# jhultman/vision3d

Hardware: AMD Instinct MI355X
Metric: frames/sec SECOND fwd, 16k-pt KITTI cloud (higher is better)
Workload: dtype f16x3-scaled (fp32-class): fp32 operands split into f16 hi + lo pieces of x * s under per-tensor power-of-two scales, 3 MFMA terms (lo*hi + hi*lo + hi*hi), fp32 accumulate; relative product error 2^-22 -- the result differs from the reference's fp32 modules by fp32 summation noise: strict elementwis

## Files before the change

### vision3d_amd/csrc/dense_conv.hip

```cpp
#include "v3d_internal.h"
#include "split_prec.h"

typedef unsigned short bf16_t;

#define DC_BM 64
#define DC_BN 128
#define DC_KC 32
#define DC_THREADS 256

template <int PREC>
__global__ void dc_pack_weights_kernel(const float* __restrict__ w, const float* __restrict__ scale, int Cout, int Cin,
                                       int ks, int CoutPad, bf16_t* __restrict__ img) {
  const int taps = ks * ks, chunks = Cin / DC_KC;
  const long long total = (long long)taps * chunks * (CoutPad / 16) * 4 * 16 * 8;
  float sw = 1.f;
  if constexpr (PREC == 1) sw = v3d_wimg_weight_scale(reinterpret_cast<unsigned*>(img + total * 2));
  for (long long t = (long long)blockIdx.x * blockDim.x + threadIdx.x; t < total; t += (long long)gridDim.x * blockDim.x) {
    long long r = t;
    const int e = (int)(r % 8); r /= 8;
    const int j = (int)(r % 16); r /= 16;
    const int kg = (int)(r % 4); r /= 4;
    const int nf = (int)(r % (CoutPad / 16)); r /= (CoutPad / 16);
    const int chunk = (int)(r % chunks); r /= chunks;
    const int tap = (int)r;
// ... 481 lines not shown
#endif
#if DL_TIMELINE
__device__ unsigned long long dl_tl[2][64];
extern "C" int v3d_debug_dense_timeline(unsigned long long* host_out) {
  return (int)hipMemcpyFromSymbol(host_out, HIP_SYMBOL(dl_tl), sizeof(dl_tl));
}
#define DL_STAMP(role, idx) do { if (blockIdx.x == 8 && lane == 0 && (wave == 0 || wave == 4)) dl_tl[role][idx] = __builtin_readcyclecounter(); } while (0)
#else
#define DL_STAMP(role, idx)
#endif

__device__ __attribute__((aligned(16))) const unsigned dl_zero16[4] = {0u, 0u, 0u, 0u};

template <int KS, int MT, int PREC>
__device__ __forceinline__ void dl_tile(unsigned char* smem_l, const bf16_t* __restrict__ x_hi, const bf16_t* __restrict__ x_lo,
                                        const bf16_t* __restrict__ w_img, const float* __restrict__ bias, const DcParams& p,
                                        bf16_t* __restrict__ y_hi, bf16_t* __restrict__ y_lo, float* __restrict__ y_nchw,
                                        const int mtile) {
  constexpr int BM = MT * 16, A_PLANE = BM * DL_KC * 2, STAGE = 2 * A_PLANE;
  const int tid = threadIdx.x, lane = tid & 63;
  const int wave = __builtin_amdgcn_readfirstlane(tid >> 6);
  const bool loader = wave >= 4;
  const int m0 = mtile * BM;
  const int n0 = blockIdx.y * DC_BN;
  if (p.occ) {
    const int R = p.reach, wpr = (p.W + 31) >> 5, span = 2 * R + 1;
    const int mlast = min(m0 + BM, p.M) - 1;
    const int r0 = m0 / p.W, r1 = mlast / p.W;
    const int per_seg = span * wpr, total = (r1 - r0 + 1) * per_seg;
    bool near_any = false;
    for (int q = lane; q < total; q += 64) {
      const int seg = q / per_seg, rem = q - seg * per_seg, dy = rem / wpr - R, wd = rem % wpr;
      const int r = r0 + seg, rr = r + dy;
      if (rr < 0 || rr >= p.B * p.H || rr / p.H != r / p.H) continue;
      const int xs = (r == r0 ? m0 - r0 * p.W : 0) - R, xe = (r == r1 ? mlast - r1 * p.W : p.W - 1) + R;
      const int lo = max(xs, wd * 32), hi = min(min(xe, p.W - 1), wd * 32 + 31);
      if (lo > hi) continue;
      const unsigned mask = (0xFFFFFFFFu >> (31 - (hi - wd * 32))) & (0xFFFFFFFFu << (lo - wd * 32));
      near_any |= (~p.occ[(size_t)rr * wpr + wd] & mask) != 0u;
    }
    if (!__builtin_amdgcn_readfirstlane(__ballot(near_any) != 0ull)) {
      if (p.tile_state) {
        if (p.tile_state[mtile] == 0u) return;
        __syncthreads();
        if (tid == 0) p.tile_state[mtile] = 0u;
      }
      const int HW = p.H * p.W, parts = (min(p.cout_store, n0 + DC_BN) - n0) >> 3;
      for (int q = tid; q < BM * parts; q += DL_THREADS) {
        const int row = q / parts, part = q - row * parts;
        const int m = m0 + row;
        if (m >= p.M) break;
        const size_t src = (size_t)(m % HW) * p.cout_store + n0 + part * 8, dst = (size_t)m * p.cout_store + n0 + part * 8;
        *reinterpret_cast<u32x4*>(y_hi + dst) = *reinterpret_cast<const u32x4*>(p.bg_hi + src);
        *reinterpret_cast<u32x4*>(y_lo + dst) = *reinterpret_cast<const u32x4*>(p.bg_lo + src);
      }
      return;
    }
  }
  if (p.tile_state && tid == 0) p.tile_state[mtile] = 1u;
  const int chunks = (p.Cin + DL_KC - 1) / DL_KC;
  const int stages = KS * KS * chunks;
  auto a_slot = [](int px, int part) { return px * 256 + ((part ^ (px & 15)) << 4); };

  f32x4 acc[MT][2];
#pragma unroll
  for (int i = 0; i < MT; i++) {
    acc[i][0] = f32x4{0.f, 0.f, 0.f, 0.f};
    acc[i][1] = f32x4{0.f, 0.f, 0.f, 0.f};
  }

  if (loader) {
    const int lw = wave - 4;
    const int sub = lane >> 4, slot = lane & 15;
    int a_pix[MT], a_hw[MT];
    {
      const int m = m0 + lw * MT * 4 + sub;
      const int b = m / (p.H * p.W), rem = m - b * p.H * p.W;
      int h = rem / p.W, w = rem - h * p.W;
#pragma unroll
      for (int j = 0; j < MT; j++) {
        const int mj = m + 4 * j;
        a_pix[j] = mj < p.M ? mj : -1;
        a_hw[j] = mj < p.M ? ((h << 16) | w) : 0;
        w += 4;
        if (w >= p.W) {
          w -= p.W;
          if (++h == p.H) h = 0;
        }
      }
    }
    typedef const __attribute__((address_space(1))) void* gptr_t;
    typedef __attribute__((address_space(3))) void* lptr_t;
    int tap = 0, chunk = 0;
    auto gather = [&](int buf) {
      const int dy = KS == 3 ? tap / 3 - 1 : 0, dx = KS == 3 ? tap % 3 - 1 : 0;
      unsigned char* A = smem_l + buf * STAGE + lw * MT * 1024;
#pragma unroll
      for (int j = 0; j < MT; j++) {
        const int px = (lw * MT + j) * 4 + sub;
        const int ch = chunk * DL_KC + ((slot ^ (px & 15)) << 3);
        const int hh = (a_hw[j] >> 16) + dy, ww = (a_hw[j] & 0xFFFF) + dx;
        const bool ok = a_pix[j] >= 0 && hh >= 0 && hh < p.H && ww >= 0 && ww < p.W && ch < p.Cin;
        const size_t off = (size_t)(a_pix[j] + dy * p.W + dx) * p.Cin + ch;
        const bf16_t* sh = ok ? x_hi + off : reinterpret_cast<const bf16_t*>(dl_zero16);
        const bf16_t* sl = ok ? x_lo + off : reinterpret_cast<const bf16_t*>(dl_zero16);
        __builtin_amdgcn_global_load_lds((gptr_t)sh, (lptr_t)(A + j * 1024), 16, 0, 0);
        __builtin_amdgcn_global_load_lds((gptr_t)sl, (lptr_t)(A + A_PLANE + j * 1024), 16, 0, 0);
      }
      if (++chunk == chunks) {
        chunk = 0;
        ++tap;
      }
    };
    DL_STAMP(1, 0);
    gather(0);
    DL_STAMP(1, 1);
    __syncthreads();
    DL_STAMP(1, 2);
    for (int s = 0; s < stages; s++) {
      if (s + 1 < stages) gather((s + 1) & 1);
      if (s < 8) DL_STAMP(1, 3 + 2 * s);
      __syncthreads();
      if (s < 8) DL_STAMP(1, 4 + 2 * s);
    }
    DL_STAMP(1, 30);
  } else {
    const size_t plane_elems = (size_t)(p.CoutPad / 16) * 4 * 16 * 8;
    u32x4 cb[DL_SS][4];
    int tap = 0, chunk = 0;
    auto load_b = [&](int ss) {
      const int steps32 = p.Cin / DC_KC;
      const size_t step = (size_t)tap * steps32 + min(chunk * DL_SS + ss, steps32 - 1);
      const bf16_t* wb = w_img + step * 2 * plane_elems + ((size_t)(n0 / 16 + wave * 2) * 64 + lane) * 8;
#pragma unroll
      for (int nt2 = 0; nt2 < 2; nt2++) {
        cb[ss][nt2 * 2 + 0] = *reinterpret_cast<const u32x4*>(wb + (size_t)nt2 * 512);
        cb[ss][nt2 * 2 + 1] = *reinterpret_cast<const u32x4*>(wb + plane_elems + (size_t)nt2 * 512);
      }
    };
    auto next_stage = [&]() {
      if (++chunk == chunks) {
        chunk = 0;
        ++tap;
      }
    };
    auto multiply = [&](int buf, bool more, bool stamp) {
      const unsigned char* A = smem_l + buf * STAGE;
      constexpr int NSTEP = DL_SS * MT / 2;
      u32x4 fh[3][2], fl[3][2];
      auto frag = [&](int t, u32x4& h, u32x4& l) {
        const int ss = t / MT, i = t % MT;
        const int off = a_slot(i * 16 + (lane & 15), ss * 4 + (lane >> 4));
        h = *reinterpret_cast<const u32x4*>(A + off);
        l = *reinterpret_cast<const u32x4*>(A + A_PLANE + off);
      };
      frag(0, fh[0][0], fl[0][0]);
      frag(1, fh[0][1], fl[0][1]);
      frag(2, fh[1][0], fl[1][0]);
      frag(3, fh[1][1], fl[1][1]);
#pragma unroll
      for (int u = 0; u < NSTEP; u++) {
        if (u + 2 < NSTEP) {
          frag(2 * u + 4, fh[(u + 2) % 3][0], fl[(u + 2) % 3][0]);
          frag(2 * u + 5, fh[(u + 2) % 3][1], fl[(u + 2) % 3][1]);
        }
        const int t0 = 2 * u, t1 = 2 * u + 1;
        const int s0 = t0 / MT, i0 = t0 % MT, s1 = t1 / MT, i1 = t1 % MT;
        const u32x4 b0h0 = cb[s0][0], b0l0 = cb[s0][1];
        const u32x4 b0h1 = cb[s0][2], b0l1 = cb[s0][3];
        const u32x4 b1h0 = cb[s1][0], b1l0 = cb[s1][1];
        const u32x4 b1h1 = cb[s1][2], b1l1 = cb[s1][3];
        const u32x4 a0h = fh[u % 3][0], a0l = fl[u % 3][0], a1h = fh[u % 3][1], a1l = fl[u % 3][1];
        acc[i0][0] = split_mfma<PREC>(a0l, b0h0, acc[i0][0]);
        acc[i0][1] = split_mfma<PREC>(a0l, b0h1, acc[i0][1]);
        acc[i1][0] = split_mfma<PREC>(a1l, b1h0, acc[i1][0]);
        acc[i1][1] = split_mfma<PREC>(a1l, b1h1, acc[i1][1]);
        __builtin_amdgcn_sched_barrier(0);
        acc[i0][0] = split_mfma<PREC>(a0h, b0l0, acc[i0][0]);
        acc[i0][1] = split_mfma<PREC>(a0h, b0l1, acc[i0][1]);
        acc[i1][0] = split_mfma<PREC>(a1h, b1l0, acc[i1][0]);
        acc[i1][1] = split_mfma<PREC>(a1h, b1l1, acc[i1][1]);
        __builtin_amdgcn_sched_barrier(0);
        acc[i0][0] = split_mfma<PREC>(a0h, b0h0, acc[i0][0]);
        acc[i0][1] = split_mfma<PREC>(a0h, b0h1, acc[i0][1]);
        acc[i1][0] = split_mfma<PREC>(a1h, b1h0, acc[i1][0]);
        acc[i1][1] = split_mfma<PREC>(a1h, b1h1, acc[i1][1]);
        if (i0 == MT - 1) load_b(s0);
        if (i1 == MT - 1) load_b(s1);
        __builtin_amdgcn_sched_barrier(0);
#if DL_TIMELINE
        if (stamp && (u == 0 || u == 1 || u == 8 || u == 16 || u == 17)) DL_STAMP(0, 40 + u);
#endif
      }
    };
    DL_STAMP(0, 0);
#pragma unroll
    for (int ss = 0; ss < DL_SS; ss++) load_b(ss);
    if (stages > 1) next_stage();
    DL_STAMP(0, 1);
    __syncthreads();
    DL_STAMP(0, 2);
    for (int s = 0; s < stages; s++) {
      const bool more = s + 1 < stages;
      multiply(s & 1, more, s == 3);
      if (s + 2 < stages) next_stage();
      if (s < 8) DL_STAMP(0, 3 + 2 * s);
      __syncthreads();
      if (s < 8) DL_STAMP(0, 4 + 2 * s);
    }
    DL_STAMP(0, 30);
  }

  DL_STAMP(loader ? 1 : 0, 31);
  const DcScales sc = dc_scales<PREC>(p);
  float vmax = 0.f;
  float* tile = reinterpret_cast<float*>(smem_l);
  f32x4 eb0 = f32x4{0.f, 0.f, 0.f, 0.f}, eb1 = eb0;
  {
    const int co = n0 + (tid & 15) * 8;
    if (bias && y_hi && co < p.cout_store) {
      eb0 = *reinterpret_cast<const f32x4*>(bias + co);
      eb1 = *reinterpret_cast<const f32x4*>(bias + co + 4);
    }
  }
  if (!loader) {
#pragma unroll
    for (int i = 0; i < MT; i++)
#pragma unroll
      for (int j = 0; j < 2; j++)
#pragma unroll
        for (int r = 0; r < 4; r++) {
          const int row = i * 16 + (lane >> 4) * 4 + r;
          const int col = wave * 32 + j * 16 + (lane & 15);
          tile[row * DL_TS + col] = acc[i][j][r];
        }
  }
  __syncthreads();
  DL_STAMP(loader ? 1 : 0, 32);
  if (y_hi) {
    const int c8 = tid & 15, co = n0 + c8 * 8;
    if (co < p.cout_store) {
#pragma unroll
      for (int k = 0; k < (BM + 31) / 32; k++) {
        const int row = (tid >> 4) + 32 * k;
        const int m = m0 + row;
        if (row < BM && m < p.M) {
          const f32x4 t0 = *reinterpret_cast<const f32x4*>(tile + row * DL_TS + c8 * 8);
          const f32x4 t1 = *reinterpret_cast<const f32x4*>(tile + row * DL_TS + c8 * 8 + 4);
          float v[8] = {dc_finish<PREC>(t0[0], eb0[0], sc), dc_finish<PREC>(t0[1], eb0[1], sc), dc_finish<PREC>(t0[2], eb0[2], sc),
                        dc_finish<PREC>(t0[3], eb0[3], sc), dc_finish<PREC>(t1[0], eb1[0], sc), dc_finish<PREC>(t1[1], eb1[1], sc),
                        dc_finish<PREC>(t1[2], eb1[2], sc), dc_finish<PREC>(t1[3], eb1[3], sc)};
          u32x4 vh, vl;
#pragma unroll
          for (int e2 = 0; e2 < 4; e2++) {
            float v0 = v[2 * e2], v1 = v[2 * e2 + 1];
            if (p.relu) {
              v0 = fmaxf(v0, 0.f);
              v1 = fmaxf(v1, 0.f);
            }
            if constexpr (PREC == 1) vmax = fmaxf(vmax, fmaxf(fabsf(v0), fabsf(v1)));
            unsigned h, l;
            split_pair<PREC>(v0, v1, sc.s_out, h, l);
            vh[e2] = h;
            vl[e2] = l;
          }
          *reinterpret_cast<u32x4*>(y_hi + (size_t)m * p.cout_store + co) = vh;
          *reinterpret_cast<u32x4*>(y_lo + (size_t)m * p.cout_store + co) = vl;
        }
      }
    }
    if constexpr (PREC == 1) dc_range_check(p, vmax, sc.limit);
  }
  if (y_nchw) {
    const int HW = p.H * p.W;
    for (int q = tid; q < (BM / 4) * DC_BN; q += DL_THREADS) {
      const int col = q / (BM / 4), r4 = q % (BM / 4);
      const int co = n0 + col;
      if (co >= p.cout_store) continue;
      const float bv = bias ? bias[co] : 0.f;
#pragma unroll
      for (int e = 0; e < 4; e++) {
        const int m = m0 + r4 * 4 + e;
        if (m >= p.M) continue;
        float v = dc_finish<PREC>(tile[(r4 * 4 + e) * DL_TS + col], bv, sc);
        if (p.relu) v = fmaxf(v, 0.f);
        const int b = m / HW, pix = m - b * HW;
        y_nchw[((size_t)b * p.cout_store + co) * HW + pix] = v;
      }
    }
  }
  DL_STAMP(loader ? 1 : 0, 33);
}

#define D2_TH 5
#define D2_TW 16
#define D2_HW (D2_TW + 2)
#define D2_HALO ((D2_TH + 2) * D2_HW)
#define D2_PIECES ((D2_HALO + 7) / 8)
#define D2_HALF (D2_PIECES * 1024)
#define D2_PLANE (2 * D2_HALF)
static_assert(2 * D2_PLANE <= dl_smem(D2_TH), "the neighbourhood image lives in the tile kernel's LDS request");
static_assert(D2_TH * 16 * DL_TS * 4 <= 2 * D2_PLANE, "the epilogue tile reuses the image's LDS");
#define D2_THREADS 256
template <int PREC>
__device__ __forceinline__ bool dl_tile2d(unsigned char* smem_l, const bf16_t* __restrict__ x_hi, const bf16_t* __restrict__ x_lo,
                                          const bf16_t* __restrict__ w_img, const float* __restrict__ bias, const DcParams& p,
                                          bf16_t* __restrict__ y_hi, bf16_t* __restrict__ y_lo, const int mtile, int* s_next) {
  constexpr int MT = D2_TH, BM = MT * 16, NT = D2_THREADS;
  const int tid = threadIdx.x, lane = tid & 63;
  const int wave = __builtin_amdgcn_readfirstlane(tid >> 6);
  const int tx_n = (p.W + D2_TW - 1) / D2_TW, ty_n = (p.H + D2_TH - 1) / D2_TH;
  const int b = mtile / (ty_n * tx_n), rt = mtile - b * ty_n * tx_n;
  const int y0 = (rt / tx_n) * D2_TH, x0 = (rt % tx_n) * D2_TW;
  if (p.occ) {
    const int R = p.reach, wpr = (p.W + 31) >> 5;
    const int ylo = max(y0 - R, 0), yhi = min(min(y0 + D2_TH - 1, p.H - 1) + R, p.H - 1);
    const int xlo = max(x0 - R, 0), xhi = min(min(x0 + D2_TW - 1, p.W - 1) + R, p.W - 1);
    const int w0 = xlo >> 5, nw = (xhi >> 5) - w0 + 1, total = (yhi - ylo + 1) * nw;
    const unsigned in_place = p.tile_state ? p.tile_state[mtile] : 1u;
    bool near_any = false;
    for (int q = lane; q < total; q += 64) {
      const int row = ylo + q / nw, wd = w0 + q % nw;
      const int lo = max(xlo, wd * 32), hi = min(xhi, wd * 32 + 31);
      const unsigned mask = (0xFFFFFFFFu >> (31 - (hi - wd * 32))) & (0xFFFFFFFFu << (lo - wd * 32));
      near_any |= (~p.occ[((size_t)b * p.H + row) * wpr + wd] & mask) != 0u;
    }
    if (!__builtin_amdgcn_readfirstlane(__ballot(near_any) != 0ull)) {
      if (p.tile_state) {
        if (in_place == 0u) return false;
        __syncthreads();
        if (tid == 0) p.tile_state[mtile] = 0u;
      }
      const int parts = p.cout_store >> 3;
      for (int q = tid; q < BM * parts; q += NT) {
        const int row = q / parts, part = q - row * parts;
        const int yy = y0 + (row >> 4), xx = x0 + (row & 15);
        if (yy >= p.H || xx >= p.W) continue;
        const size_t src = ((size_t)yy * p.W + xx) * p.cout_store + part * 8, dst = (((size_t)b * p.H + yy) * p.W + xx) * p.cout_store + part * 8;
        *reinterpret_cast<u32x4*>(y_hi + dst) = *reinterpret_cast<const u32x4*>(p.bg_hi + src);
        *reinterpret_cast<u32x4*>(y_lo + dst) = *reinterpret_cast<const u32x4*>(p.bg_lo + src);
      }
      return false;
    }
  }
  if (p.tile_state && tid == 0) p.tile_state[mtile] = 1u;

  f32x4 acc[MT][2];
#pragma unroll
  for (int i = 0; i < MT; i++) {
    acc[i][0] = f32x4{0.f, 0.f, 0.f, 0.f};
    acc[i][1] = f32x4{0.f, 0.f, 0.f, 0.f};
  }
  {
    const int plane = wave & 1, half = wave >> 1;
    const int sub = lane >> 3, slot = lane & 7;
    const bf16_t* xp = plane ? x_lo : x_hi;
    typedef const __attribute__((address_space(1))) void* gptr_t;
    typedef __attribute__((address_space(3))) void* lptr_t;
    unsigned char* dstb = smem_l + plane * D2_PLANE + half * D2_HALF;
#pragma unroll
    for (int j = 0; j < D2_PIECES; j++) {
      const int hp = j * 8 + sub;
      const int hy = hp / D2_HW, hx = hp - hy * D2_HW;
      const int yy = y0 - 1 + hy, xx = x0 - 1 + hx;
      const bool ok = hp < D2_HALO && yy >= 0 && yy < p.H && xx >= 0 && xx < p.W;
      const int part = half * 8 + (slot ^ (hp & 7));
      const bf16_t* src = ok ? xp + (((size_t)b * p.H + yy) * p.W + xx) * p.Cin + part * 8 : reinterpret_cast<const bf16_t*>(dl_zero16);
      __builtin_amdgcn_global_load_lds((gptr_t)src, (lptr_t)(dstb + j * 1024), 16, 0, 0);
    }
  }
  {
    const size_t plane_elems = (size_t)(p.CoutPad / 16) * 4 * 16 * 8;
    u32x4 cb[DL_SS][4];
    int tapn = 0;
    auto load_b = [&](int ss) {
      const size_t step = (size_t)min(tapn, 8) * DL_SS + ss;
      const bf16_t* wb = w_img + step * 2 * plane_elems + ((size_t)(wave * 2) * 64 + lane) * 8;
#pragma unroll
      for (int nt2 = 0; nt2 < 2; nt2++) {
        cb[ss][nt2 * 2 + 0] = *reinterpret_cast<const u32x4*>(wb + (size_t)nt2 * 512);
        cb[ss][nt2 * 2 + 1] = *reinterpret_cast<const u32x4*>(wb + plane_elems + (size_t)nt2 * 512);
      }
    };
    typedef const __attribute__((address_space(3))) unsigned char* lds_t;
    const lds_t lds = (lds_t)smem_l;
    const int pxl = lane & 15, kg = lane >> 4;
    unsigned pw[8];
#pragma unroll
    for (int j = 0; j < 8; j++) pw[j] = (unsigned)(pxl * 128 + ((kg ^ ((pxl + j) & 7)) << 4));
    auto multiply = [&](auto tapc) {
      constexpr int TAP = decltype(tapc)::value;
      constexpr int dyc = TAP / 3, dxc = TAP % 3;
      constexpr int NSTEP = DL_SS * MT / 2;
      u32x4 fh[3][2], fl[3][2];
      auto frag = [&](auto tc, u32x4& h, u32x4& l) {
        constexpr int t = decltype(tc)::value;
        constexpr int ss = t / MT, i = t % MT;
        constexpr int c = (i + dyc) * D2_HW + dxc;
        const unsigned a = (pw[c & 7] ^ (unsigned)((ss & 1) << 6)) + (unsigned)((ss >> 1) * D2_HALF + c * 128);
        h = *reinterpret_cast<const __attribute__((address_space(3))) u32x4*>(lds + a);
        l = *reinterpret_cast<const __attribute__((address_space(3))) u32x4*>(lds + a + D2_PLANE);
      };
#define D2_IC(v) std::integral_constant<int, (v)>{}
      frag(D2_IC(0), fh[0][0], fl[0][0]);
      frag(D2_IC(1), fh[0][1], fl[0][1]);
      frag(D2_IC(2), fh[1][0], fl[1][0]);
      frag(D2_IC(3), fh[1][1], fl[1][1]);
      auto step = [&](auto uc) {
        constexpr int u = decltype(uc)::value;
        if constexpr (u + 2 < NSTEP) {
          frag(D2_IC(2 * u + 4), fh[(u + 2) % 3][0], fl[(u + 2) % 3][0]);
          frag(D2_IC(2 * u + 5), fh[(u + 2) % 3][1], fl[(u + 2) % 3][1]);
        }
        constexpr int t0 = 2 * u, t1 = 2 * u + 1;
        constexpr int s0 = t0 / MT, i0 = t0 % MT, s1 = t1 / MT, i1 = t1 % MT;
        const u32x4 b0h0 = cb[s0][0], b0l0 = cb[s0][1];
        const u32x4 b0h1 = cb[s0][2], b0l1 = cb[s0][3];
        const u32x4 b1h0 = cb[s1][0], b1l0 = cb[s1][1];
        const u32x4 b1h1 = cb[s1][2], b1l1 = cb[s1][3];
        const u32x4 a0h = fh[u % 3][0], a0l = fl[u % 3][0], a1h = fh[u % 3][1], a1l = fl[u % 3][1];
        acc[i0][0] = split_mfma<PREC>(a0l, b0h0, acc[i0][0]);
        acc[i0][1] = split_mfma<PREC>(a0l, b0h1, acc[i0][1]);
        acc[i1][0] = split_mfma<PREC>(a1l, b1h0, acc[i1][0]);
        acc[i1][1] = split_mfma<PREC>(a1l, b1h1, acc[i1][1]);
        __builtin_amdgcn_sched_barrier(0);
        acc[i0][0] = split_mfma<PREC>(a0h, b0l0, acc[i0][0]);
        acc[i0][1] = split_mfma<PREC>(a0h, b0l1, acc[i0][1]);
        acc[i1][0] = split_mfma<PREC>(a1h, b1l0, acc[i1][0]);
        acc[i1][1] = split_mfma<PREC>(a1h, b1l1, acc[i1][1]);
        __builtin_amdgcn_sched_barrier(0);
        acc[i0][0] = split_mfma<PREC>(a0h, b0h0, acc[i0][0]);
        acc[i0][1] = split_mfma<PREC>(a0h, b0h1, acc[i0][1]);
        acc[i1][0] = split_mfma<PREC>(a1h, b1h0, acc[i1][0]);
        acc[i1][1] = split_mfma<PREC>(a1h, b1h1, acc[i1][1]);
        if constexpr (i0 == MT - 1) load_b(s0);
        if constexpr (i1 == MT - 1) load_b(s1);
        __builtin_amdgcn_sched_barrier(0);
      };
      step(D2_IC(0)); step(D2_IC(1)); step(D2_IC(2)); step(D2_IC(3)); step(D2_IC(4));
      step(D2_IC(5)); step(D2_IC(6)); step(D2_IC(7)); step(D2_IC(8)); step(D2_IC(9));
      static_assert(NSTEP == 10, "the steps are written out");
    };
#pragma unroll
    for (int ss = 0; ss < DL_SS; ss++) load_b(ss);
    tapn = 1;
    __syncthreads();
    multiply(D2_IC(0)); tapn = 2;
    multiply(D2_IC(1)); tapn = 3;
    multiply(D2_IC(2)); tapn = 4;
    multiply(D2_IC(3)); tapn = 5;
    multiply(D2_IC(4)); tapn = 6;
    multiply(D2_IC(5)); tapn = 7;
    multiply(D2_IC(6)); tapn = 8;
    multiply(D2_IC(7));
    multiply(D2_IC(8));
#undef D2_IC
  }
  __syncthreads();
  const bool draws = s_next != nullptr && p.work != nullptr;
  unsigned drawn = 0u;
  if (draws && tid == 0) drawn = gridDim.x + atomicAdd(p.work, 1u);
  const DcScales sc = dc_scales<PREC>(p);
  float vmax = 0.f;
  float* tile = reinterpret_cast<float*>(smem_l);
  f32x4 eb0 = f32x4{0.f, 0.f, 0.f, 0.f}, eb1 = eb0;
  {
    const int co = (tid & 15) * 8;
    if (bias && co < p.cout_store) {
      eb0 = *reinterpret_cast<const f32x4*>(bias + co);
      eb1 = *reinterpret_cast<const f32x4*>(bias + co + 4);
    }
  }
#pragma unroll
  for (int i = 0; i < MT; i++)
#pragma unroll
    for (int j = 0; j < 2; j++)
#pragma unroll
      for (int r = 0; r < 4; r++) tile[(i * 16 + (lane >> 4) * 4 + r) * DL_TS + wave * 32 + j * 16 + (lane & 15)] = acc[i][j][r];
  __syncthreads();
  const int c8 = tid & 15, co = c8 * 8;
  if (co < p.cout_store) {
#pragma unroll
    for (int k = 0; k < (BM + NT / 16 - 1) / (NT / 16); k++) {
      const int row = (tid >> 4) + (NT / 16) * k;
      const int yy = y0 + (row >> 4), xx = x0 + (row & 15);
      if (row < BM && yy < p.H && xx < p.W) {
        const size_t m = ((size_t)b * p.H + yy) * p.W + xx;
        const f32x4 t0 = *reinterpret_cast<const f32x4*>(tile + row * DL_TS + c8 * 8);
        const f32x4 t1 = *reinterpret_cast<const f32x4*>(tile + row * DL_TS + c8 * 8 + 4);
        float v[8] = {dc_finish<PREC>(t0[0], eb0[0], sc), dc_finish<PREC>(t0[1], eb0[1], sc), dc_finish<PREC>(t0[2], eb0[2], sc),
                      dc_finish<PREC>(t0[3], eb0[3], sc), dc_finish<PREC>(t1[0], eb1[0], sc), dc_finish<PREC>(t1[1], eb1[1], sc),
                      dc_finish<PREC>(t1[2], eb1[2], sc), dc_finish<PREC>(t1[3], eb1[3], sc)};
        u32x4 vh, vl;
#pragma unroll
        for (int e2 = 0; e2 < 4; e2++) {
          float v0 = v[2 * e2], v1 = v[2 * e2 + 1];
          if (p.relu) {
            v0 = fmaxf(v0, 0.f);
            v1 = fmaxf(v1, 0.f);
          }
          if constexpr (PREC == 1) vmax = fmaxf(vmax, fmaxf(fabsf(v0), fabsf(v1)));
          unsigned h, l;
          split_pair<PREC>(v0, v1, sc.s_out, h, l);
          vh[e2] = h;
          vl[e2] = l;
        }
        *reinterpret_cast<u32x4*>(y_hi + m * p.cout_store + co) = vh;
        *reinterpret_cast<u32x4*>(y_lo + m * p.cout_store + co) = vl;
      }
    }
  }
  if constexpr (PREC == 1) dc_range_check(p, vmax, sc.limit);
  if (draws && tid == 0) *s_next = (int)drawn;
  return draws;
}

template <int PREC>
__global__ __launch_bounds__(D2_THREADS, 2) void conv2d_bf16x3_tile2d_kernel(const bf16_t* __restrict__ x_hi, const bf16_t* __restrict__ x_lo,
                                                                          const bf16_t* __restrict__ w_img, const float* __restrict__ bias,
                                                                          const DcParams p, bf16_t* __restrict__ y_hi,
                                                                          bf16_t* __restrict__ y_lo) {
  extern __shared__ __attribute__((aligned(16))) unsigned char smem_l[];
  __shared__ int s_next;
  const int ntiles = p.B * ((p.H + D2_TH - 1) / D2_TH) * ((p.W + D2_TW - 1) / D2_TW);
  if (p.reset_ptr && blockIdx.x == 0)
    for (int i = threadIdx.x; i < p.reset_words; i += D2_THREADS) p.reset_ptr[i] = 0u;
  for (int mtile = blockIdx.x; mtile < ntiles;) {
    const bool drew = dl_tile2d<PREC>(smem_l, x_hi, x_lo, w_img, bias, p, y_hi, y_lo, mtile, &s_next);
    if (!drew && threadIdx.x == 0) s_next = (int)(gridDim.x + atomicAdd(p.work, 1u));
    __syncthreads();
    mtile = s_next;
    __syncthreads();
  }
  if (!p.reset_ptr && threadIdx.x == 0 && atomicAdd(p.work + 1, 1u) == gridDim.x - 1) {
    p.work[0] = 0u;
    p.work[1] = 0u;
  }
}

template <int KS, int MT, int PREC>
__global__ __launch_bounds__(DL_THREADS) void conv2d_bf16x3_large_kernel(const bf16_t* __restrict__ x_hi,
                                                                         const bf16_t* __restrict__ x_lo,
                                                                         const bf16_t* __restrict__ w_img,
                                                                         const float* __restrict__ bias, const DcParams p,
                                                                         bf16_t* __restrict__ y_hi, bf16_t* __restrict__ y_lo,
                                                                         float* __restrict__ y_nchw) {
  extern __shared__ __attribute__((aligned(16))) unsigned char smem_l[];
  __shared__ int s_next;
  if (!p.work) {
    const int nt = gridDim.x;
    int mtile = blockIdx.x;
    {
      const int q = nt / 8, rmd = nt % 8, xcd = mtile % 8, idx = mtile / 8;
      mtile = (xcd < rmd ? xcd * (q + 1) : rmd * (q + 1) + (xcd - rmd) * q) + idx;
    }
    dl_tile<KS, MT, PREC>(smem_l, x_hi, x_lo, w_img, bias, p, y_hi, y_lo, y_nchw, mtile);
    return;
  }
  const int ntiles = (p.M + MT * 16 - 1) / (MT * 16);
  if (p.reset_ptr && blockIdx.x == 0)
    for (int i = threadIdx.x; i < p.reset_words; i += DL_THREADS) p.reset_ptr[i] = 0u;
  for (int mtile = blockIdx.x; mtile < ntiles;) {
    dl_tile<KS, MT, PREC>(smem_l, x_hi, x_lo, w_img, bias, p, y_hi, y_lo, y_nchw, mtile);
    if (threadIdx.x == 0) s_next = (int)(gridDim.x + atomicAdd(p.work, 1u));
    __syncthreads();
    mtile = s_next;
    __syncthreads();
  }
  if (!p.reset_ptr && threadIdx.x == 0 && atomicAdd(p.work + 1, 1u) == gridDim.x - 1) {
    p.work[0] = 0u;
    p.work[1] = 0u;
  }
}

template <int STEPS, int PREC>
__global__ __launch_bounds__(256) void conv1x1_bf16x3_small_cout_kernel(const bf16_t* __restrict__ x_hi,
                                                                        const bf16_t* __restrict__ x_lo,
                                                                        const bf16_t* __restrict__ w_img,
                                                                        const float* __restrict__ bias, const DcParams p,
                                                                        float* __restrict__ y_nchw) {
  const int lane = threadIdx.x & 63, wave = threadIdx.x >> 6;
  const int m0 = (blockIdx.x * 4 + wave) * 16;
  if (m0 >= p.M) return;
  const size_t plane_elems = (size_t)(p.CoutPad / 16) * 4 * 16 * 8;
  const int px = min(m0 + (lane & 15), p.M - 1);
  const bf16_t* xh = x_hi + (size_t)px * p.Cin + (lane >> 4) * 8;
  const bf16_t* xl = x_lo + (size_t)px * p.Cin + (lane >> 4) * 8;
  const bf16_t* wb = w_img + (size_t)lane * 8;
  u32x4 bh[STEPS], bl[STEPS], ah[STEPS], al[STEPS];
#pragma unroll
  for (int s = 0; s < STEPS; s++) {
      bh[s] = *reinterpret_cast<const u32x4*>(wb + (size_t)s * 2 * plane_elems);
      bl[s] = *reinterpret_cast<const u32x4*>(wb + (size_t)s * 2 * plane_elems + plane_elems);
      ah[s] = *reinterpret_cast<const u32x4*>(xh + s * DC_KC);
      al[s] = *reinterpret_cast<const u32x4*>(xl + s * DC_KC);
    }
  f32x4 c_lh = {0.f, 0.f, 0.f, 0.f}, c_hl = c_lh, c_hh = c_lh;
#pragma unroll
  for (int s = 0; s < STEPS; s++) {
      c_lh = split_mfma<PREC>(al[s], bh[s], c_lh);
      c_hl = split_mfma<PREC>(ah[s], bl[s], c_hl);
      c_hh = split_mfma<PREC>(ah[s], bh[s], c_hh);
    }
  const int co = lane & 15;
  if (co >= p.cout_store) return;
  const DcScales sc = dc_scales<PREC>(p);
  const float bv = bias ? bias[co] : 0.f;
  const int HW = p.H * p.W;
#pragma unroll
  for (int r = 0; r < 4; r++) {
    const int m = m0 + (lane >> 4) * 4 + r;
    if (m >= p.M) continue;
    float v = dc_finish<PREC>((c_lh[r] + c_hl[r]) + c_hh[r], bv, sc);
    if (p.relu) v = fmaxf(v, 0.f);
    const int b = m / HW, pix = m - b * HW;
    y_nchw[((size_t)b * p.cout_store + co) * HW + pix] = v;
  }
}

#define FH_WAVES 9
#define FH_ROW 272
#define FH_SLAB (2 * 16 * FH_ROW)
#define FH_W1_BYTES (4 * 2 * 128 * 32 * 2)
#define FH_SMEM (FH_W1_BYTES + FH_WAVES * FH_SLAB)
struct FhScales {
  const float *in_entry, *mid_entry, *w1_inv, *w2_inv;
  int* range_flag;
};
template <int PREC>
__global__ __launch_bounds__(FH_WAVES * 64) void conv1x1_head_fused_kernel(const bf16_t* __restrict__ x_hi, const bf16_t* __restrict__ x_lo,
                                                                          const bf16_t* __restrict__ w1_img, const float* __restrict__ b1,
                                                                          int relu1, const bf16_t* __restrict__ w2_img,
                                                                          const float* __restrict__ b2, int relu2, int M, int HW,
                                                                          int cout2, int cout2_pad, float* __restrict__ y_nchw,
                                                                          const FhScales fs) {
  extern __shared__ __attribute__((aligned(16))) unsigned char fh_smem[];
  const int tid = threadIdx.x, lane = tid & 63;
  const int wave = __builtin_amdgcn_readfirstlane(tid >> 6);
  {
    const u32x4* src = reinterpret_cast<const u32x4*>(w1_img);
    u32x4* dst = reinterpret_cast<u32x4*>(fh_smem);
    for (int i = tid; i < FH_W1_BYTES / 16; i += FH_WAVES * 64) dst[i] = src[i];
  }
  u32x4 h_bh[4], h_bl[4];
  {
    const size_t pe2 = (size_t)cout2_pad * 32;
#pragma unroll
    for (int s = 0; s < 4; s++) {
      h_bh[s] = *reinterpret_cast<const u32x4*>(w2_img + (size_t)s * 2 * pe2 + (size_t)lane * 8);
      h_bl[s] = *reinterpret_cast<const u32x4*>(w2_img + (size_t)s * 2 * pe2 + pe2 + (size_t)lane * 8);
    }
  }
  __syncthreads();
  DcScales sc1{1.f, 1.f, 3.0e38f}, sc2{1.f, 1.f, 3.0e38f};
  if constexpr (PREC == 1) {
    sc1.undo = fs.in_entry[1] * fs.w1_inv[0];
    sc1.s_out = fs.mid_entry[0];
    sc1.limit = fs.mid_entry[2];
    sc2.undo = fs.mid_entry[1] * fs.w2_inv[0];
  }
  float vmax = 0.f;
  const unsigned char* w1s = fh_smem;
  unsigned char* slab = fh_smem + FH_W1_BYTES + wave * FH_SLAB;
  const int px_l = lane & 15, kg = lane >> 4;
  const int ntiles = (M + 15) / 16;
  for (int t = blockIdx.x * FH_WAVES + wave; t < ntiles; t += gridDim.x * FH_WAVES) {
    const int m0 = t * 16;
    const int px = min(m0 + px_l, M - 1);
    u32x4 ah[4], al[4];
#pragma unroll
    for (int s = 0; s < 4; s++) {
      ah[s] = *reinterpret_cast<const u32x4*>(x_hi + (size_t)px * 128 + s * 32 + kg * 8);
      al[s] = *reinterpret_cast<const u32x4*>(x_lo + (size_t)px * 128 + s * 32 + kg * 8);
    }
    f32x4 acc[8];
#pragma unroll
    for (int nf = 0; nf < 8; nf++) acc[nf] = f32x4{0.f, 0.f, 0.f, 0.f};
#pragma unroll
    for (int s = 0; s < 4; s++) {
      u32x4 bh[8], bl[8];
#pragma unroll
      for (int nf = 0; nf < 8; nf++) {
        bh[nf] = *reinterpret_cast<const u32x4*>(w1s + s * 16384 + (nf * 64 + lane) * 16);
        bl[nf] = *reinterpret_cast<const u32x4*>(w1s + s * 16384 + 8192 + (nf * 64 + lane) * 16);
      }
      const u32x4 a_h = ah[s], a_l = al[s];
#pragma unroll
      for (int nf = 0; nf < 8; nf++) acc[nf] = split_mfma<PREC>(a_l, bh[nf], acc[nf]);
#pragma unroll
      for (int nf = 0; nf < 8; nf++) acc[nf] = split_mfma<PREC>(a_h, bl[nf], acc[nf]);
#pragma unroll
      for (int nf = 0; nf < 8; nf++) acc[nf] = split_mfma<PREC>(a_h, bh[nf], acc[nf]);
    }
#pragma unroll
    for (int nf = 0; nf < 8; nf++) {
      const float bv = b1 ? b1[nf * 16 + px_l] : 0.f;
#pragma unroll
      for (int r2 = 0; r2 < 2; r2++) {
        float v0 = dc_finish<PREC>(acc[nf][2 * r2], bv, sc1), v1 = dc_finish<PREC>(acc[nf][2 * r2 + 1], bv, sc1);
        if (relu1) {
          v0 = fmaxf(v0, 0.f);
          v1 = fmaxf(v1, 0.f);
        }
        if constexpr (PREC == 1) vmax = fmaxf(vmax, fmaxf(fabsf(v0), fabsf(v1)));
        unsigned h, l;
        split_pair<PREC>(v0, v1, sc1.s_out, h, l);
        const int p0 = kg * 4 + 2 * r2, off = (nf * 16 + px_l) * 2;
        *reinterpret_cast<unsigned short*>(slab + p0 * FH_ROW + off) = (unsigned short)(h & 0xFFFFu);
        *reinterpret_cast<unsigned short*>(slab + (p0 + 1) * FH_ROW + off) = (unsigned short)(h >> 16);
        *reinterpret_cast<unsigned short*>(slab + 16 * FH_ROW + p0 * FH_ROW + off) = (unsigned short)(l & 0xFFFFu);
        *reinterpret_cast<unsigned short*>(slab + 16 * FH_ROW + (p0 + 1) * FH_ROW + off) = (unsigned short)(l >> 16);
      }
    }
    asm volatile("s_waitcnt lgkmcnt(0)" ::: "memory");
    f32x4 c_lh = {0.f, 0.f, 0.f, 0.f}, c_hl = c_lh, c_hh = c_lh;
#pragma unroll
    for (int s = 0; s < 4; s++) {
      const u32x4 a2h = *reinterpret_cast<const u32x4*>(slab + px_l * FH_ROW + s * 64 + kg * 16);
      const u32x4 a2l = *reinterpret_cast<const u32x4*>(slab + 16 * FH_ROW + px_l * FH_ROW + s * 64 + kg * 16);
      c_lh = split_mfma<PREC>(a2l, h_bh[s], c_lh);
      c_hl = split_mfma<PREC>(a2h, h_bl[s], c_hl);
      c_hh = split_mfma<PREC>(a2h, h_bh[s], c_hh);
    }
    asm volatile("s_waitcnt lgkmcnt(0)" ::: "memory");
    const int co = px_l;
    if (co < cout2) {
      const float bv = b2 ? b2[co] : 0.f;
#pragma unroll
      for (int r = 0; r < 4; r++) {
        const int m = m0 + kg * 4 + r;
        if (m >= M) continue;
        float v = dc_finish<PREC>((c_lh[r] + c_hl[r]) + c_hh[r], bv, sc2);
        if (relu2) v = fmaxf(v, 0.f);
        const int b = m / HW, pix = m - b * HW;
        y_nchw[((size_t)b * cout2 + co) * HW + pix] = v;
      }
    }
  }
  if constexpr (PREC == 1)
    if (fs.range_flag && vmax > sc1.limit) atomicMax(fs.range_flag, V3D_FLAG_RANGE);
}

static int dc_check_prec(const v3d_conv2d_prec* pr, bool planes_out) {
  if (!pr || pr->prec == V3D_PREC_BF16X3) return V3D_OK;
  if (pr->prec != V3D_PREC_F16S || !pr->in_entry || (planes_out && !pr->out_entry)) return V3D_EINVAL;
  return V3D_OK;
}

extern "C" int v3d_conv2d_1x1_head_fused(const void* x_hi, const void* x_lo, const void* w1_image, const float* b1, int relu1,
                                          const void* w2_image, const float* b2, int relu2, int B, int H, int W, int Cmid, int Cout2,
                                          float* y_nchw, const v3d_conv2d_prec* pr, v3d_stream_t stream) {
  if (!x_hi || !x_lo || !w1_image || !w2_image || !y_nchw || B < 1 || H < 1 || W < 1) return V3D_EINVAL;
  if (Cmid != 128 || Cout2 < 1 || Cout2 > 16) return V3D_EUNSUPPORTED;
  if (dc_check_prec(pr, true)) return V3D_EINVAL;
  const int n_cu = v3d_device_cu_count();
  if (n_cu < 1) return V3D_EINVAL;
  const int M = B * H * W, ntiles = (M + 15) / 16;
  const int grid = std::min(v3d_ceil_div(ntiles, FH_WAVES), n_cu);
  const int cout2_pad = (Cout2 + DC_BN - 1) / DC_BN * DC_BN;
  const bool f16s = pr && pr->prec == V3D_PREC_F16S;
  FhScales fs{nullptr, nullptr, nullptr, nullptr, nullptr};
  if (f16s) {
    fs.in_entry = pr->in_entry;
    fs.mid_entry = pr->out_entry;
    fs.w1_inv = pr->w_inv ? pr->w_inv : reinterpret_cast<const float*>(reinterpret_cast<const char*>(w1_image) + dc_image_payload_bytes(128, 128, 1)) + V3D_WIMG_INV_SCALE;
    fs.w2_inv = pr->w_inv2 ? pr->w_inv2 : reinterpret_cast<const float*>(reinterpret_cast<const char*>(w2_image) + dc_image_payload_bytes(128, Cout2, 1)) + V3D_WIMG_INV_SCALE;
    fs.range_flag = pr->range_flag;
  }
  auto kern = f16s ? conv1x1_head_fused_kernel<1> : conv1x1_head_fused_kernel<0>;
  V3D_CHECK_HIP(hipFuncSetAttribute((const void*)kern, hipFuncAttributeMaxDynamicSharedMemorySize, FH_SMEM));
  hipLaunchKernelGGL(kern, dim3(grid), dim3(FH_WAVES * 64), FH_SMEM, (hipStream_t)stream, (const bf16_t*)x_hi,
                     (const bf16_t*)x_lo, (const bf16_t*)w1_image, b1, relu1, (const bf16_t*)w2_image, b2, relu2, M, H * W, Cout2,
                     cout2_pad, y_nchw, fs);
  V3D_CHECK_LAUNCH();
  return V3D_OK;
}

extern "C" int v3d_conv2d_bg_tiles(int B, int H, int W);
__global__ __launch_bounds__(V3D_BLOCK) void bev_occupancy_kernel(const int4* __restrict__ coords, const int* __restrict__ n_ptr,
                                                                  int cap, int H, int W, unsigned* __restrict__ occ) {
  const int n = min(*n_ptr, cap), wpr = (W + 31) >> 5;
  for (int i = blockIdx.x * V3D_BLOCK + threadIdx.x; i < n; i += gridDim.x * V3D_BLOCK) {
    const int4 c = coords[i];
    atomicAnd(occ + ((size_t)c.x * H + c.z) * wpr + (c.w >> 5), ~(1u << (c.w & 31)));
  }
}

extern "C" size_t v3d_bev_occupancy_words(int B, int H, int W) { return (size_t)B * H * ((W + 31) >> 5); }

extern "C" int v3d_bev_occupancy_bits(const int32_t* coords, const int32_t* n, int cap, int B, int H, int W, uint32_t* occ,
                                      v3d_stream_t stream) {
  if (!coords || !n || !occ || cap < 1 || B < 1 || H < 1 || W < 1) return V3D_EINVAL;
  hipStream_t st = (hipStream_t)stream;
  V3D_CHECK_HIP(v3d_fill_async(occ, 0xFF, v3d_bev_occupancy_words(B, H, W) * sizeof(uint32_t), st));
  hipLaunchKernelGGL(bev_occupancy_kernel, dim3(std::min(v3d_ceil_div(cap, V3D_BLOCK), 1024)), dim3(V3D_BLOCK), 0, st,
                     (const int4*)coords, n, cap, H, W, occ);
  V3D_CHECK_LAUNCH();
  return V3D_OK;
}

extern "C" int v3d_conv2d_bg_tiles(int B, int H, int W) {
  const long long flat = ((long long)B * H * W + 5 * 16 - 1) / (5 * 16);
  const long long blocks = (long long)B * ((H + D2_TH - 1) / D2_TH) * ((W + D2_TW - 1) / D2_TW);
  return (int)(flat > blocks ? flat : blocks);
}

template <int PREC>
static int dc_launch(const void* x_hi, const void* x_lo, const void* weight_image, const float* bias, DcParams p, int ksize,
                     void* y_hi, void* y_lo, float* y_nchw, const uint32_t* occ, uint32_t* work, uint32_t* tile_state,
                     uint32_t* reset_ptr, int reset_words, hipStream_t st) {
  const int B = p.B, H = p.H, W = p.W, Cin = p.Cin, Cout = p.Cout;
  if (ksize == 1 && !y_hi && Cout <= 16 && (Cin == 128 || Cin == 256)) {
    const dim3 sgrid(v3d_ceil_div(v3d_ceil_div(p.M, 16), 4));
    if (Cin == 128)
      hipLaunchKernelGGL((conv1x1_bf16x3_small_cout_kernel<4, PREC>), sgrid, dim3(256), 0, st, (const bf16_t*)x_hi, (const bf16_t*)x_lo,
                         (const bf16_t*)weight_image, bias, p, y_nchw);
    else
      hipLaunchKernelGGL((conv1x1_bf16x3_small_cout_kernel<8, PREC>), sgrid, dim3(256), 0, st, (const bf16_t*)x_hi, (const bf16_t*)x_lo,
                         (const bf16_t*)weight_image, bias, p, y_nchw);
    V3D_CHECK_LAUNCH();
    if (reset_ptr) V3D_CHECK_HIP(v3d_fill_async(reset_ptr, 0, (size_t)reset_words * 4, st));
    return V3D_OK;
  }
  const bool large_ok = Cin >= 64 && H < 32768 && W < 65536 && W >= 16;
  if (large_ok && Cout > 32) {
    const int n_cu = v3d_device_cu_count();
    if (n_cu < 1) return V3D_EINVAL;
    const bool persistent = p.occ && work && p.CoutPad == DC_BN;
    if (persistent && ksize == 3 && Cin == DL_KC) {
      if (v3d_ablate('d')) return V3D_OK;
      p.work = work;
// ... 83 lines not shown
```

Measured before the change: 4773.

## Compact live pixels per tile in 2D conv and skip background rows

Builds a per-row bitmask of output pixels that lie within reach of occupied cells, using a bit-window dilation with shuffles when the reach is small. Only those pixels are packed into a compacted list in LDS and fed through the MFMA loop in 16-row blocks; the remaining pixels are filled from the precomputed background image in the epilogue. This is meant to cut MFMA and LDS work on partially empty tiles, at the cost of extra mask logic, indirect LDS addressing and several extra template instantiations. Weight-load addressing is also reworked to use a byte offset computed once per lane.

```diff
diff --git a/vision3d_amd/csrc/dense_conv.hip b/vision3d_amd/csrc/dense_conv.hip
--- a/vision3d_amd/csrc/dense_conv.hip
+++ b/vision3d_amd/csrc/dense_conv.hip
@@ -807,28 +807,55 @@
 static_assert(2 * D2_PLANE <= dl_smem(D2_TH), "the neighbourhood image lives in the tile kernel's LDS request");
 static_assert(D2_TH * 16 * DL_TS * 4 <= 2 * D2_PLANE, "the epilogue tile reuses the image's LDS");
 #define D2_THREADS 256
+#define D2_RMAX 24
 template <int PREC>
 __device__ __forceinline__ bool dl_tile2d(unsigned char* smem_l, const bf16_t* __restrict__ x_hi, const bf16_t* __restrict__ x_lo,
                                           const bf16_t* __restrict__ w_img, const float* __restrict__ bias, const DcParams& p,
-                                          bf16_t* __restrict__ y_hi, bf16_t* __restrict__ y_lo, const int mtile, int* s_next) {
+                                          bf16_t* __restrict__ y_hi, bf16_t* __restrict__ y_lo, const int mtile, int* s_next,
+                                          unsigned char* s_list) {
   constexpr int MT = D2_TH, BM = MT * 16, NT = D2_THREADS;
-  const int tid = threadIdx.x, lane = tid & 63;
+  int tid_ = threadIdx.x;
+  asm volatile("" : "+v"(tid_));
+  const int tid = tid_, lane = tid & 63;
   const int wave = __builtin_amdgcn_readfirstlane(tid >> 6);
   const int tx_n = (p.W + D2_TW - 1) / D2_TW, ty_n = (p.H + D2_TH - 1) / D2_TH;
   const int b = mtile / (ty_n * tx_n), rt = mtile - b * ty_n * tx_n;
   const int y0 = (rt / tx_n) * D2_TH, x0 = (rt % tx_n) * D2_TW;
+  const unsigned in_cols = x0 + D2_TW <= p.W ? 0xFFFFu : (1u << (p.W - x0)) - 1u;
+  unsigned rm[MT];
+#pragma unroll
+  for (int ty = 0; ty < MT; ty++) rm[ty] = y0 + ty < p.H ? in_cols : 0u;
   if (p.occ) {
     const int R = p.reach, wpr = (p.W + 31) >> 5;
-    const int ylo = max(y0 - R, 0), yhi = min(min(y0 + D2_TH - 1, p.H - 1) + R, p.H - 1);
-    const int xlo = max(x0 - R, 0), xhi = min(min(x0 + D2_TW - 1, p.W - 1) + R, p.W - 1);
-    const int w0 = xlo >> 5, nw = (xhi >> 5) - w0 + 1, total = (yhi - ylo + 1) * nw;
     const unsigned in_place = p.tile_state ? p.tile_state[mtile] : 1u;
     bool near_any = false;
-    for (int q = lane; q < total; q += 64) {
-      const int row = ylo + q / nw, wd = w0 + q % nw;
-      const int lo = max(xlo, wd * 32), hi = min(xhi, wd * 32 + 31);
-      const unsigned mask = (0xFFFFFFFFu >> (31 - (hi - wd * 32))) & (0xFFFFFFFFu << (lo - wd * 32));
-      near_any |= (~p.occ[((size_t)b * p.H + row) * wpr + wd] & mask) != 0u;
+    unsigned long long win = 0ull;
+    if (R <= D2_RMAX) {
+      const int y = y0 - R + lane, cs = x0 - R, wi0 = cs >> 5, sh = cs & 31;
+      if (lane < D2_TH + 2 * R && y >= 0 && y < p.H) {
+        const unsigned* rowp = p.occ + ((size_t)b * p.H + y) * wpr;
+        unsigned w[3];
+#pragma unroll
+        for (int k = 0; k < 3; k++) {
+          const int wi = wi0 + k;
+          w[k] = (wi >= 0 && wi < wpr) ? ~rowp[wi] : 0u;
+          if (wi == wpr - 1 && (p.W & 31)) w[k] &= (1u << (p.W & 31)) - 1u;
+        }
+        win = (((unsigned long long)w[1] << 32) | w[0]) >> sh;
+        if (sh) win |= (unsigned long long)w[2] << (64 - sh);
+        if (D2_TW + 2 * R < 64) win &= (1ull << (D2_TW + 2 * R)) - 1ull;
+      }
+      near_any = win != 0ull;
+    } else {
+      const int ylo = max(y0 - R, 0), yhi = min(min(y0 + D2_TH - 1, p.H - 1) + R, p.H - 1);
+      const int xlo = max(x0 - R, 0), xhi = min(min(x0 + D2_TW - 1, p.W - 1) + R, p.W - 1);
+      const int w0 = xlo >> 5, nw = (xhi >> 5) - w0 + 1, total = (yhi - ylo + 1) * nw;
+      for (int q = lane; q < total; q += 64) {
+        const int row = ylo + q / nw, wd = w0 + q % nw;
+        const int lo = max(xlo, wd * 32), hi = min(xhi, wd * 32 + 31);
+        const unsigned mask = (0xFFFFFFFFu >> (31 - (hi - wd * 32))) & (0xFFFFFFFFu << (lo - wd * 32));
+        near_any |= (~p.occ[((size_t)b * p.H + row) * wpr + wd] & mask) != 0u;
+      }
     }
     if (!__builtin_amdgcn_readfirstlane(__ballot(near_any) != 0ull)) {
       if (p.tile_state) {
@@ -847,7 +874,23 @@
       }
       return false;
     }
-  }
+    if (R <= D2_RMAX) {
+      const int L = 2 * R + 1;
+      int len = 1;
+      for (; 2 * len <= L; len *= 2) win |= win >> len;
+      win |= win >> (L - len);
+      unsigned v = (unsigned)win & in_cols;
+      for (len = 1; 2 * len <= L; len *= 2) v |= (unsigned)__shfl_down((int)v, len);
+      v |= (unsigned)__shfl_down((int)v, L - len);
+#pragma unroll
+      for (int ty = 0; ty < MT; ty++) rm[ty] &= (unsigned)__builtin_amdgcn_readlane((int)v, ty);
+    }
+  }
+  int pre[MT + 1];
+  pre[0] = 0;
+#pragma unroll
+  for (int ty = 0; ty < MT; ty++) pre[ty + 1] = pre[ty] + __builtin_popcount(rm[ty]);
+  const int n_live = pre[MT], nb = (n_live + 15) >> 4;
   if (p.tile_state && tid == 0) p.tile_state[mtile] = 1u;
 
   f32x4 acc[MT][2];
@@ -874,17 +917,31 @@
       __builtin_amdgcn_global_load_lds((gptr_t)src, (lptr_t)(dstb + j * 1024), 16, 0, 0);
     }
   }
+  const bool whole = n_live == BM;
+  if (!whole && tid < BM) {
+    const int ty = tid >> 4, x = tid & 15;
+    const unsigned m = ty == 0 ? rm[0] : ty == 1 ? rm[1] : ty == 2 ? rm[2] : ty == 3 ? rm[3] : rm[4];
+    const int at = (ty == 0 ? pre[0] : ty == 1 ? pre[1] : ty == 2 ? pre[2] : ty == 3 ? pre[3] : pre[4]) + __builtin_popcount(m & ((1u << x) - 1u));
+    if ((m >> x) & 1u) s_list[at] = (unsigned char)tid;
+    if (tid >= n_live && tid < 16 * nb) {
+      const int fy = rm[0] ? 0 : rm[1] ? 1 : rm[2] ? 2 : rm[3] ? 3 : 4;
+      const unsigned fm = rm[0] ? rm[0] : rm[1] ? rm[1] : rm[2] ? rm[2] : rm[3] ? rm[3] : rm[4];
+      s_list[tid] = (unsigned char)(fy * 16 + __builtin_ctz(fm));
+    }
+  }
+  static_assert(MT == 5, "the row selects are written out");
   {
     const size_t plane_elems = (size_t)(p.CoutPad / 16) * 4 * 16 * 8;
     u32x4 cb[DL_SS][4];
     int tapn = 0;
+    const unsigned wlane = (unsigned)(((wave * 2) * 64 + lane) * 8 * (int)sizeof(bf16_t));
     auto load_b = [&](int ss) {
       const size_t step = (size_t)min(tapn, 8) * DL_SS + ss;
-      const bf16_t* wb = w_img + step * 2 * plane_elems + ((size_t)(wave * 2) * 64 + lane) * 8;
+      const unsigned char* wb = reinterpret_cast<const unsigned char*>(w_img + step * 2 * plane_elems);
 #pragma unroll
       for (int nt2 = 0; nt2 < 2; nt2++) {
-        cb[ss][nt2 * 2 + 0] = *reinterpret_cast<const u32x4*>(wb + (size_t)nt2 * 512);
-        cb[ss][nt2 * 2 + 1] = *reinterpret_cast<const u32x4*>(wb + plane_elems + (size_t)nt2 * 512);
+        cb[ss][nt2 * 2 + 0] = *reinterpret_cast<const u32x4*>(wb + nt2 * 1024 + wlane);
+        cb[ss][nt2 * 2 + 1] = *reinterpret_cast<const u32x4*>(wb + plane_elems * sizeof(bf16_t) + nt2 * 1024 + wlane);
       }
     };
     typedef const __attribute__((address_space(3))) unsigned char* lds_t;
@@ -946,19 +1003,112 @@
       step(D2_IC(5)); step(D2_IC(6)); step(D2_IC(7)); step(D2_IC(8)); step(D2_IC(9));
       static_assert(NSTEP == 10, "the steps are written out");
     };
+    auto compact = [&](auto nbc) {
+      constexpr int NB = decltype(nbc)::value, NSTEP = DL_SS * NB / 2;
+      unsigned hp0[NB];
+#pragma unroll
+      for (int j = 0; j < NB; j++) {
+        const unsigned q = s_list[16 * j + pxl];
+        hp0[j] = (q >> 4) * D2_HW + (q & 15u);
+      }
+#pragma unroll 1
+      for (int tap = 0; tap < 9; tap++) {
+        tapn = tap + 1;
+        const unsigned toff = (unsigned)((tap / 3) * D2_HW + tap % 3);
+        u32x4 fh[3][2], fl[3][2];
+        auto frag = [&](auto tc, u32x4& h, u32x4& l) {
+          constexpr int t = decltype(tc)::value;
+          constexpr int ss = t / NB, i = t % NB;
+          const unsigned hp = hp0[i] + toff;
+          const unsigned a = ((hp << 7) | ((((unsigned)kg ^ hp) & 7u) << 4)) ^ (unsigned)((ss & 1) << 6);
+          h = *reinterpret_cast<const __attribute__((address_space(3))) u32x4*>(lds + a + (ss >> 1) * D2_HALF);
+          l = *reinterpret_cast<const __attribute__((address_space(3))) u32x4*>(lds + a + (ss >> 1) * D2_HALF + D2_PLANE);
+        };
+        frag(D2_IC(0), fh[0][0], fl[0][0]);
+        frag(D2_IC(1), fh[0][1], fl[0][1]);
+        if constexpr (NSTEP > 1) {
+          frag(D2_IC(2), fh[1][0], fl[1][0]);
+          frag(D2_IC(3), fh[1][1], fl[1][1]);
+        }
+        auto step = [&](auto uc) {
+          constexpr int u = decltype(uc)::value;
+          if constexpr (u < NSTEP) {
+            if constexpr (u + 2 < NSTEP) {
+              frag(D2_IC(2 * u + 4), fh[(u + 2) % 3][0], fl[(u + 2) % 3][0]);
+              frag(D2_IC(2 * u + 5), fh[(u + 2) % 3][1], fl[(u + 2) % 3][1]);
+            }
+            constexpr int t0 = 2 * u, t1 = 2 * u + 1;
+            constexpr int s0 = t0 / NB, i0 = t0 % NB, s1 = t1 / NB, i1 = t1 % NB;
+            const u32x4 b0h0 = cb[s0][0], b0l0 = cb[s0][1];
+            const u32x4 b0h1 = cb[s0][2], b0l1 = cb[s0][3];
+            const u32x4 b1h0 = cb[s1][0], b1l0 = cb[s1][1];
+            const u32x4 b1h1 = cb[s1][2], b1l1 = cb[s1][3];
+            const u32x4 a0h = fh[u % 3][0], a0l = fl[u % 3][0], a1h = fh[u % 3][1], a1l = fl[u % 3][1];
+            if constexpr (i0 == i1) {
+              acc[i0][0] = split_mfma<PREC>(a0l, b0h0, acc[i0][0]);
+              acc[i0][1] = split_mfma<PREC>(a0l, b0h1, acc[i0][1]);
+              acc[i0][0] = split_mfma<PREC>(a0h, b0l0, acc[i0][0]);
+              acc[i0][1] = split_mfma<PREC>(a0h, b0l1, acc[i0][1]);
+              acc[i0][0] = split_mfma<PREC>(a0h, b0h0, acc[i0][0]);
+              acc[i0][1] = split_mfma<PREC>(a0h, b0h1, acc[i0][1]);
+              __builtin_amdgcn_sched_barrier(0);
+              acc[i1][0] = split_mfma<PREC>(a1l, b1h0, acc[i1][0]);
+              acc[i1][1] = split_mfma<PREC>(a1l, b1h1, acc[i1][1]);
+              acc[i1][0] = split_mfma<PREC>(a1h, b1l0, acc[i1][0]);
+              acc[i1][1] = split_mfma<PREC>(a1h, b1l1, acc[i1][1]);
+              acc[i1][0] = split_mfma<PREC>(a1h, b1h0, acc[i1][0]);
+              acc[i1][1] = split_mfma<PREC>(a1h, b1h1, acc[i1][1]);
+            } else {
+              acc[i0][0] = split_mfma<PREC>(a0l, b0h0, acc[i0][0]);
+              acc[i0][1] = split_mfma<PREC>(a0l, b0h1, acc[i0][1]);
+              acc[i1][0] = split_mfma<PREC>(a1l, b1h0, acc[i1][0]);
+              acc[i1][1] = split_mfma<PREC>(a1l, b1h1, acc[i1][1]);
+              __builtin_amdgcn_sched_barrier(0);
+              acc[i0][0] = split_mfma<PREC>(a0h, b0l0, acc[i0][0]);
+              acc[i0][1] = split_mfma<PREC>(a0h, b0l1, acc[i0][1]);
+              acc[i1][0] = split_mfma<PREC>(a1h, b1l0, acc[i1][0]);
+              acc[i1][1] = split_mfma<PREC>(a1h, b1l1, acc[i1][1]);
+              __builtin_amdgcn_sched_barrier(0);
+              acc[i0][0] = split_mfma<PREC>(a0h, b0h0, acc[i0][0]);
+              acc[i0][1] = split_mfma<PREC>(a0h, b0h1, acc[i0][1]);
+              acc[i1][0] = split_mfma<PREC>(a1h, b1h0, acc[i1][0]);
+              acc[i1][1] = split_mfma<PREC>(a1h, b1h1, acc[i1][1]);
+            }
+            if constexpr (i0 == NB - 1) load_b(s0);
+            if constexpr (i1 == NB - 1) load_b(s1);
+            __builtin_amdgcn_sched_barrier(0);
+          }
+        };
+        step(D2_IC(0)); step(D2_IC(1)); step(D2_IC(2)); step(D2_IC(3)); step(D2_IC(4));
+        step(D2_IC(5)); step(D2_IC(6)); step(D2_IC(7)); step(D2_IC(8)); step(D2_IC(9));
+        static_assert(NSTEP <= 10, "the steps are written out");
+      }
+    };
 #pragma unroll
     for (int ss = 0; ss < DL_SS; ss++) load_b(ss);
     tapn = 1;
     __syncthreads();
-    multiply(D2_IC(0)); tapn = 2;
-    multiply(D2_IC(1)); tapn = 3;
-    multiply(D2_IC(2)); tapn = 4;
-    multiply(D2_IC(3)); tapn = 5;
-    multiply(D2_IC(4)); tapn = 6;
-    multiply(D2_IC(5)); tapn = 7;
-    multiply(D2_IC(6)); tapn = 8;
-    multiply(D2_IC(7));
-    multiply(D2_IC(8));
+    if (whole) {
+      multiply(D2_IC(0)); tapn = 2;
+      multiply(D2_IC(1)); tapn = 3;
+      multiply(D2_IC(2)); tapn = 4;
+      multiply(D2_IC(3)); tapn = 5;
+      multiply(D2_IC(4)); tapn = 6;
+      multiply(D2_IC(5)); tapn = 7;
+      multiply(D2_IC(6)); tapn = 8;
+      multiply(D2_IC(7));
+      multiply(D2_IC(8));
+    } else if (nb == 1) {
+      compact(D2_IC(1));
+    } else if (nb == 2) {
+      compact(D2_IC(2));
+    } else if (nb == 3) {
+      compact(D2_IC(3));
+    } else if (nb == 4) {
+      compact(D2_IC(4));
+    } else {
+      compact(D2_IC(5));
+    }
 #undef D2_IC
   }
   __syncthreads();
@@ -978,19 +1128,28 @@
   }
 #pragma unroll
   for (int i = 0; i < MT; i++)
-#pragma unroll
-    for (int j = 0; j < 2; j++)
-#pragma unroll
-      for (int r = 0; r < 4; r++) tile[(i * 16 + (lane >> 4) * 4 + r) * DL_TS + wave * 32 + j * 16 + (lane & 15)] = acc[i][j][r];
+    if (i < nb) {
+#pragma unroll
+      for (int j = 0; j < 2; j++)
+#pragma unroll
+        for (int r = 0; r < 4; r++) tile[(i * 16 + (lane >> 4) * 4 + r) * DL_TS + wave * 32 + j * 16 + (lane & 15)] = acc[i][j][r];
+    }
   __syncthreads();
   const int c8 = tid & 15, co = c8 * 8;
   if (co < p.cout_store) {
-#pragma unroll
-    for (int k = 0; k < (BM + NT / 16 - 1) / (NT / 16); k++) {
-      const int row = (tid >> 4) + (NT / 16) * k;
-      const int yy = y0 + (row >> 4), xx = x0 + (row & 15);
-      if (row < BM && yy < p.H && xx < p.W) {
-        const size_t m = ((size_t)b * p.H + yy) * p.W + xx;
+    static_assert(NT / 16 == D2_TW && BM / D2_TW == MT, "one tile row per pass");
+#pragma unroll
+    for (int k = 0; k < MT; k++) {
+      const int xl = tid >> 4;
+      const int yy = y0 + k, xx = x0 + xl;
+      if (yy >= p.H || xx >= p.W) continue;
+      const size_t m = ((size_t)b * p.H + yy) * p.W + xx;
+      if (!((rm[k] >> xl) & 1u)) {
+        const size_t src = ((size_t)yy * p.W + xx) * p.cout_store + co;
+        *reinterpret_cast<u32x4*>(y_hi + m * p.cout_store + co) = *reinterpret_cast<const u32x4*>(p.bg_hi + src);
+        *reinterpret_cast<u32x4*>(y_lo + m * p.cout_store + co) = *reinterpret_cast<const u32x4*>(p.bg_lo + src);
+      } else {
+        const int row = pre[k] + __builtin_popcount(rm[k] & ((1u << xl) - 1u));
         const f32x4 t0 = *reinterpret_cast<const f32x4*>(tile + row * DL_TS + c8 * 8);
         const f32x4 t1 = *reinterpret_cast<const f32x4*>(tile + row * DL_TS + c8 * 8 + 4);
         float v[8] = {dc_finish<PREC>(t0[0], eb0[0], sc), dc_finish<PREC>(t0[1], eb0[1], sc), dc_finish<PREC>(t0[2], eb0[2], sc),
@@ -1027,11 +1186,12 @@
                                                                           bf16_t* __restrict__ y_lo) {
   extern __shared__ __attribute__((aligned(16))) unsigned char smem_l[];
   __shared__ int s_next;
+  __shared__ unsigned char s_list[D2_TH * D2_TW];
   const int ntiles = p.B * ((p.H + D2_TH - 1) / D2_TH) * ((p.W + D2_TW - 1) / D2_TW);
   if (p.reset_ptr && blockIdx.x == 0)
     for (int i = threadIdx.x; i < p.reset_words; i += D2_THREADS) p.reset_ptr[i] = 0u;
   for (int mtile = blockIdx.x; mtile < ntiles;) {
-    const bool drew = dl_tile2d<PREC>(smem_l, x_hi, x_lo, w_img, bias, p, y_hi, y_lo, mtile, &s_next);
+    const bool drew = dl_tile2d<PREC>(smem_l, x_hi, x_lo, w_img, bias, p, y_hi, y_lo, mtile, &s_next, s_list);
     if (!drew && threadIdx.x == 0) s_next = (int)(gridDim.x + atomicAdd(p.work, 1u));
     __syncthreads();
     mtile = s_next;
```

Result: no change. 4779 (median of 2 runs) (+0.1%).
